# fskovbo/OptimalControlMPS

Hardware: NVIDIA B200
Metric: cost+gradient evals/s (BH N=20 chi=100) (higher is better)
Workload: dtype complex128 (f64)

## Files before the change

optimalcontrolmps_b200/csrc/decomp.cu:

```cuda
#include <cstdio>
#include <cstdlib>
#include "ocmps_internal.h"

__device__ unsigned long long g_jac_dbg[8];
__device__ double g_jac_flops[2];

namespace {

constexpr int JAC_THREADS = 512;
constexpr int JAC_EPL = 8;
constexpr int JAC_NV_SMEM = 512;
constexpr int JAC_MAX_SWEEPS = 60;
constexpr int JAC_BLOCKED_ROWS = 64;
constexpr double JAC_TOL2 = 1e-28;
constexpr double DEFLATE_REL = 1e-30;
constexpr int NV_MAX = 2048;
constexpr int BJ_C = 8;
constexpr int BJ_TPP = 4;
constexpr int BJ_MAX_ROWS = 256;
constexpr int BJ_SLOTS = BJ_MAX_ROWS / 2;
constexpr int BJ_THREADS = BJ_SLOTS * BJ_TPP;
constexpr int BJ_MAX_EPL = 8;
constexpr int BJ_MIN_CAP = 112;

// ... 1837 lines not shown
    }
#ifdef OCMPS_JAC_TRACE
    if (nv >= 24)
      printf("JTR kind %d blk %d nv %d keff %d rb %d jac %lld : rotation rounds %d, %lld clk per round; block exchanges %d, %lld clk each\n", a.kind, blk, nv,
             keff, rb, t_jac1 - t_jac0, nrounds, nrounds ? t_work / nrounds : 0ll, nxchg, nxchg ? t_xchg / nxchg : 0ll);
#endif
  }
}

__global__ void __launch_bounds__(JAC_THREADS) jacobi_rows_cluster_kernel(DecompArgs a, DecompBuffers b, int smem_elems) {
  extern __shared__ __align__(16) unsigned char smem_raw[];
  __shared__ RcShared sh;
  const int blk = (int)blockIdx.x / RC_C;
  const unsigned rank = clus::cluster_rank();
  const int keff = rot_handover_rows(b, blk, smem_elems);
  if (keff < 0) return;
  if (keff < RC_MIN_ROWS) {
    if (rank == 0) jacobi_rot_block(a, b, blk, keff, smem_raw);
    return;
  }
  cplx* Zs = reinterpret_cast<cplx*>(smem_raw);
  switch ((b.dw->blk[blk].nv + 15) >> 4) {
    case 1: rc_run<1>(a, b, blk, keff, rank, Zs, sh); break;
    case 2: rc_run<2>(a, b, blk, keff, rank, Zs, sh); break;
    case 3: rc_run<3>(a, b, blk, keff, rank, Zs, sh); break;
    case 4: rc_run<4>(a, b, blk, keff, rank, Zs, sh); break;
    case 5: rc_run<5>(a, b, blk, keff, rank, Zs, sh); break;
    case 6: rc_run<6>(a, b, blk, keff, rank, Zs, sh); break;
    case 7: rc_run<7>(a, b, blk, keff, rank, Zs, sh); break;
    default: rc_run<8>(a, b, blk, keff, rank, Zs, sh); break;
  }
}

__global__ void __launch_bounds__(1024) truncate_kernel(DecompArgs a, DecompBuffers b, TruncParams tp) {
  __shared__ double cP[NV_MAX];
  __shared__ double sSorted[NV_MAX];
  __shared__ short cQ[NV_MAX], cI[NV_MAX], cI2[NV_MAX];
  __shared__ unsigned char sKeep[NV_MAX];
  __shared__ int sBlkOff[OCMPS_MAX_BLK + 1];
  __shared__ double sWarp[32];
  __shared__ int sWarpCnt[33];
  __shared__ double s_docut, s_kept;
  __shared__ int s_nfinal;
  DecompWork* w = b.dw;
  const int nv = w->nvtot;
  const int nblocks = w->nblocks;
  const int tid = threadIdx.x, lane = tid & 31, warp = tid >> 5;
  for (int i = tid; i < nblocks; i += blockDim.x) sBlkOff[i] = w->blk[i].p_off;
  if (tid == 0) { s_nfinal = 0; s_docut = 0.0; }
  const int i0 = 2 * tid, i1 = i0 + 1;
  const double p0 = i0 < nv ? b.P[i0] : 0.0, p1 = i1 < nv ? b.P[i1] : 0.0;
  const int f0 = p0 > 0.0, f1 = p1 > 0.0;
  int incl = f0 + f1;
#pragma unroll
  for (int o = 1; o < 32; o <<= 1) { const int up = __shfl_up_sync(0xffffffffu, incl, o); if (lane >= o) incl += up; }
  if (lane == 31) sWarpCnt[warp + 1] = incl;
  if (tid == 0) sWarpCnt[0] = 0;
  __syncthreads();
  if (warp == 0) {
    int v = sWarpCnt[lane + 1];
#pragma unroll
    for (int o = 1; o < 32; o <<= 1) { const int up = __shfl_up_sync(0xffffffffu, v, o); if (lane >= o) v += up; }
    sWarpCnt[lane + 1] = v;
  }
  __syncthreads();
  const int nnz = sWarpCnt[32];
  {
    int k = sWarpCnt[warp] + incl - f0 - f1;
    if (f0) { cP[k] = p0; cQ[k] = (short)b.vecq[i0]; cI[k] = (short)i0; ++k; }
    if (f1) { cP[k] = p1; cQ[k] = (short)b.vecq[i1]; cI[k] = (short)i1; }
  }
  __syncthreads();
  {
    int tpe = 1;
    while (tpe < 8 && nnz * tpe * 2 <= (int)blockDim.x) tpe *= 2;
    const int sub = tid & (tpe - 1);
    for (int k0 = 0; k0 < nnz; k0 += (int)blockDim.x / tpe) {
      const int k = k0 + tid / tpe;
      const bool in = k < nnz;
      const double pk = in ? cP[k] : 0.0;
      int rank = 0;
      if (in)
        for (int j = sub; j < nnz; j += tpe) {
          const double pj = cP[j];
          rank += (pj > pk) || (pj == pk && j < k);
        }
      for (int o = 1; o < tpe; o <<= 1) rank += __shfl_xor_sync(0xffffffffu, rank, o);
      if (in && sub == 0) sSorted[rank] = pk;
    }
  }
  __syncthreads();
  const int origm = nv;
  const int e0 = nnz - 1 - 2 * tid, e1 = e0 - 1;
  const double v0 = e0 >= 0 ? sSorted[e0] : 0.0, v1 = e1 >= 0 ? sSorted[e1] : 0.0;
  {
    double run = v0 + v1;
#pragma unroll
    for (int o = 1; o < 32; o <<= 1) { const double up = __shfl_up_sync(0xffffffffu, run, o); if (lane >= o) run += up; }
    if (lane == 31) sWarp[warp] = run;
    __syncthreads();
    if (warp == 0) {
      double ws = sWarp[lane];
#pragma unroll
// ... 17 lines not shown
      best = nmax > 0 ? nmax : 0;
    } else {
      const int lim = nmax < nnz - 1 ? nmax : nnz - 1;
      for (int n = tid; n <= lim; n += blockDim.x)
        if (n < tp.minm || sSorted[n] >= cut) best = n > best ? n : best;
      if (tp.minm - 1 > best && tp.minm - 1 <= nmax) best = tp.minm - 1;
    }
    if (best > 0) atomicMax(&s_nfinal, best);
  }
  __syncthreads();
  {
    const int m = s_nfinal + 1;
    if (tid == 0) { sWarp[0] = 0.0; sWarp[1] = 0.0; }
    __syncthreads();
    if (e0 == m) sWarp[0] = v0;
    if (e1 == m) sWarp[0] = v1;
    if (e0 == m - 1) sWarp[1] = v0;
    if (e1 == m - 1) sWarp[1] = v1;
    __syncthreads();
    if (tid == 0) {
      double docut = 0.0;
      if (origm == 1) {
        docut = sWarp[1] / 2.0;
      } else if (origm > 1 && m < origm) {
        const double pm = sWarp[0], pm1 = sWarp[1];
        docut = (pm + pm1) / 2.0;
        if (fabs(pm - pm1) < 1e-3 * pm1) docut += 1e-3 * pm1;
      }
      s_docut = docut;
    }
    __syncthreads();
  }
  const double docut = s_docut;
  {
    const int ka = 2 * tid, kb = ka + 1;
    const int fa = ka < nnz && cP[ka] > docut, fb = kb < nnz && cP[kb] > docut;
    if (ka < nnz) sKeep[ka] = (unsigned char)fa;
    if (kb < nnz) sKeep[kb] = (unsigned char)fb;
    int inc = fa + fb;
#pragma unroll
    for (int o = 1; o < 32; o <<= 1) { const int up = __shfl_up_sync(0xffffffffu, inc, o); if (lane >= o) inc += up; }
    __syncthreads();
    if (lane == 31) sWarpCnt[warp + 1] = inc;
    if (tid == 0) sWarpCnt[0] = 0;
    __syncthreads();
    if (warp == 0) {
      int v = sWarpCnt[lane + 1];
#pragma unroll
      for (int o = 1; o < 32; o <<= 1) { const int up = __shfl_up_sync(0xffffffffu, v, o); if (lane >= o) v += up; }
      sWarpCnt[lane + 1] = v;
    }
    __syncthreads();
    const int base = sWarpCnt[warp] + inc - fa - fb;
    if (ka < nnz) cI2[ka] = (short)base;
    if (kb < nnz) cI2[kb] = (short)(base + fa);
  }
  __syncthreads();
  const int total = sWarpCnt[32];
  int* inv_blk = b.pos + NV_MAX;
  int* inv_v = b.pos + 2 * NV_MAX;
  double part = 0.0;
  for (int k = tid; k < nnz; k += blockDim.x) {
    if (!sKeep[k]) continue;
    const int qk = cQ[k];
    const double pk = cP[k];
    int rank = 0, j = k - 1;
    for (; j >= 0 && cQ[j] == qk; --j) rank += sKeep[j] && cP[j] >= pk;
    const int pos0 = cI2[j + 1];
    for (j = k + 1; j < nnz && cQ[j] == qk; ++j) rank += sKeep[j] && cP[j] > pk;
    const int pos = pos0 + rank;
    if (pos < tp.cap) {
      const int i = cI[k];
      a.qNew[pos] = qk;
      int bi = 0;
      while (bi + 1 < nblocks && sBlkOff[bi + 1] <= i) ++bi;
      inv_blk[pos] = bi;
      inv_v[pos] = i - sBlkOff[bi];
      part += pk;
    }
  }
  {
#pragma unroll
    for (int o = 16; o > 0; o >>= 1) part += __shfl_xor_sync(0xffffffffu, part, o);
    __syncthreads();
    if (lane == 0) sWarp[warp] = part;
    __syncthreads();
    if (tid == 0) {
      double t = 0.0;
      for (int i = 0; i < 32; ++i) t += sWarp[i];
      s_kept = t;
    }
    __syncthreads();
  }
  if (tid == 0) {
    int k = total;
    if (k == 0 && nv > 0) {
      k = 1;
      a.qNew[0] = b.vecq[0];
      inv_blk[0] = 0;
      inv_v[0] = 0;
    }
    if (k > tp.cap) { atomicOr(b.status, OCMPS_ST_CAPACITY); k = tp.cap; }
    w->newdim = k;
    *a.dimNew = k;
    const double kept = s_kept;
    double scale = 1.0;
    if (tp.normalize) {
      const double nrm = sqrt(kept);
      if (nrm > 1e-16) scale = 1.0 / nrm;
    }
    w->scale = scale;
    const int n = w->n, m = w->m;
    GemmDesc g1;
    g1.pad = 0;
    g1.A = g1.B = nullptr; g1.C = nullptr; g1.M = g1.N = g1.K = 0; g1.lda = g1.ldb = g1.ldc = 1; g1.opA = g1.opB = 0;
    if (a.kind == DK_ORTH_LEFT) {
      const int far = a.D * (*a.dimNb);
      g1.A = a.partner; g1.opA = 0; g1.lda = m;
      g1.B = a.nb_in; g1.opB = 0; g1.ldb = far;
      g1.C = a.nb_out; g1.ldc = far; g1.M = k; g1.N = far; g1.K = m;
    } else if (a.kind == DK_ORTH_RIGHT) {
      const int far = a.D * (*a.dimNb);
      g1.A = a.nb_in; g1.opA = 0; g1.lda = n;
      g1.B = a.partner; g1.opB = 0; g1.ldb = k;
      g1.C = a.nb_out; g1.ldc = k; g1.M = far; g1.N = k; g1.K = n;
    }
    b.descs[1] = g1;
  }
}

constexpr int BUILD_THREADS = 512;
__global__ void __launch_bounds__(BUILD_THREADS) build_factors_kernel(DecompArgs a, DecompBuffers b) {
  extern __shared__ __align__(16) unsigned char bsm[];
  __shared__ double red[BUILD_THREADS / 32];
  __shared__ double s_inv;
  const DecompWork* w = b.dw;
  const int k = w->newdim;
  const int kk = blockIdx.x;
  if (kk >= k) return;
  const int n = w->n, m = w->m, ld = w->ld, mode = w->mode;
  const int* comp_blk = b.comp_idx + NV_MAX;
  const int* comp_rank = b.comp_idx + 2 * NV_MAX;
  const int* vec_blk = b.vec_idx + NV_MAX;
  const int* vec_rank = b.vec_idx + 2 * NV_MAX;
  const int bi = b.pos[NV_MAX + kk], j = b.pos[2 * NV_MAX + kk];
  const DecompBlock B = w->blk[bi];
  const int nv = B.nv, len = B.len;
  const cplx* Zj = b.ywork + B.ws_off + (size_t)j * nv;
  const double sigma = sqrt(b.P[B.p_off + j]) * w->scale;
  cplx* zs = reinterpret_cast<cplx*>(bsm);
  cplx* out = zs + nv;
  int* vidx = reinterpret_cast<int*>(out + len);
  int* cidx = vidx + nv;
  const int tid = threadIdx.x, lane = tid & 31, wp = tid >> 5;
  constexpr int NW = BUILD_THREADS / 32;
  for (int v = tid; v < nv; v += BUILD_THREADS) { zs[v] = Zj[v]; vidx[v] = b.vec_idx[B.vec_off + v]; }
  for (int c = tid; c < len; c += BUILD_THREADS) cidx[c] = b.comp_idx[B.comp_off + c];
  __syncthreads();
  double part = 0.0;
  if (mode == 0) {
    for (int c = wp; c < len; c += NW) {
      const cplx* row = a.X + (size_t)cidx[c] * ld;
      double sr = 0.0, si = 0.0;
      for (int v0 = 0; v0 < nv; v0 += 128) {
        cplx x[4];
#pragma unroll
        for (int u = 0; u < 4; ++u) {
          const int v = v0 + lane + 32 * u;
          x[u] = make_double2(0.0, 0.0);
          if (v < nv) x[u] = row[vidx[v]];
        }
#pragma unroll
        for (int u = 0; u < 4; ++u) {
          const int v = v0 + lane + 32 * u;
          if (v < nv) {
            const cplx z = zs[v];
            sr += x[u].x * z.x + x[u].y * z.y;
            si += x[u].y * z.x - x[u].x * z.y;
          }
        }
      }
      sr = warp_sum(sr); si = warp_sum(si);
      if (lane == 0) { out[c] = make_double2(sr, si); part += sr * sr + si * si; }
    }
  } else {
    const int cl = lane & 7, g = lane >> 3;
    for (int c0 = 8 * wp; c0 < len; c0 += 8 * NW) {
      const int c = c0 + cl;
      const bool in = c < len;
      const cplx* colp = a.X + (in ? cidx[c] : 0);
      double sr = 0.0, si = 0.0;
      if (in) {
#pragma unroll 4
        for (int v = g; v < nv; v += 4) {
          const cplx x = colp[(size_t)vidx[v] * ld], z = zs[v];
          sr += x.x * z.x + x.y * z.y;
          si += x.y * z.x - x.x * z.y;
        }
      }
      sr += __shfl_xor_sync(0xffffffffu, sr, 8);  si += __shfl_xor_sync(0xffffffffu, si, 8);
      sr += __shfl_xor_sync(0xffffffffu, sr, 16); si += __shfl_xor_sync(0xffffffffu, si, 16);
      if (in && g == 0) { out[c] = make_double2(sr, si); part += sr * sr + si * si; }
    }
  }
  part = warp_sum(part);
  if ((tid & 31) == 0) red[tid >> 5] = part;
  __syncthreads();
  if (tid == 0) {
    double t = 0.0;
    for (int i = 0; i < BUILD_THREADS / 32; ++i) t += red[i];
    s_inv = t > 0.0 ? rsqrt(t) : 0.0;
  }
  __syncthreads();
  const double inv = s_inv;
  const int ncomp = mode == 0 ? n : m, nvec = mode == 0 ? m : n;
  for (int c = tid; c < ncomp; c += BUILD_THREADS) {
    cplx v = make_double2(0.0, 0.0);
    if (comp_blk[c] == bi) { const cplx o = out[comp_rank[c]]; v = make_double2(o.x * inv, o.y * inv); }
    if (mode == 0) a.iso[(size_t)c * k + kk] = v; else a.iso[(size_t)kk * m + c] = v;
  }
  if (a.qNb != nullptr && (a.kind == DK_ORTH_LEFT || a.kind == DK_ORTH_RIGHT)) {
    const int D = a.D, chiFar = *a.dimNb, qj = B.q;
    if (a.kind == DK_ORTH_LEFT) {
      const long long far = (long long)D * chiFar;
      for (int r = tid; r < chiFar; r += BUILD_THREADS) {
        const int sx = a.qNb[r] - qj;
        double ar = 0.0, ai = 0.0;
        if (sx >= 0 && sx < D) {
          const cplx* col = a.nb_in + (long long)sx * chiFar + r;
#pragma unroll 4
          for (int t = 0; t < nv; ++t) {
            const cplx z = zs[t], x = col[(long long)vidx[t] * far];
            ar += z.x * x.x - z.y * x.y;
            ai += z.x * x.y + z.y * x.x;
          }
        }
        for (int sp = 0; sp < D; ++sp)
          a.nb_out[(long long)kk * far + (long long)sp * chiFar + r] = sp == sx ? make_double2(ar * sigma, ai * sigma) : make_double2(0.0, 0.0);
      }
    } else {
      for (int l = tid; l < chiFar; l += BUILD_THREADS) {
        const int sx = qj - a.qNb[l];
        double ar = 0.0, ai = 0.0;
        if (sx >= 0 && sx < D) {
          const cplx* row = a.nb_in + ((long long)l * D + sx) * n;
#pragma unroll 4
          for (int t = 0; t < nv; ++t) {
            const cplx z = zs[t], x = row[vidx[t]];
            ar += z.x * x.x - z.y * x.y;
            ai += z.x * x.y + z.y * x.x;
          }
        }
        for (int sp = 0; sp < D; ++sp)
          a.nb_out[((long long)l * D + sp) * k + kk] = sp == sx ? make_double2(ar * sigma, ai * sigma) : make_double2(0.0, 0.0);
      }
    }
    return;
  }
  for (int v = tid; v < nvec; v += BUILD_THREADS) {
    cplx o = make_double2(0.0, 0.0);
    if (vec_blk[v] == bi) { const cplx z = zs[vec_rank[v]]; o = make_double2(z.x * sigma, z.y * sigma); }
    if (mode == 0) a.partner[(size_t)kk * m + v] = o; else a.partner[(size_t)v * k + kk] = o;
  }
}

constexpr int NORM_CTAS = 32;
constexpr int NORM_THREADS = 256;

__device__ __forceinline__ void norm_partial_body(const cplx* x, long long count, double* partial) {
  __shared__ double red[NORM_THREADS];
  double s = 0.0;
  for (long long e = blockIdx.x * (long long)NORM_THREADS + threadIdx.x; e < count; e += (long long)NORM_CTAS * NORM_THREADS) {
    cplx u = x[e];
    s += u.x * u.x + u.y * u.y;
  }
  red[threadIdx.x] = s;
  __syncthreads();
  for (int o = NORM_THREADS / 2; o > 0; o >>= 1) {
    if ((int)threadIdx.x < o) red[threadIdx.x] += red[threadIdx.x + o];
    __syncthreads();
  }
  if (threadIdx.x == 0) partial[blockIdx.x] = red[0];
}
__device__ __forceinline__ double norm_total(const double* partial) {
  double s = 0.0;
  for (int i = 0; i < NORM_CTAS; ++i) s += partial[i];
  return s;
// ... 198 lines not shown
```

optimalcontrolmps_b200/csrc/engine.cu:

```cuda
#include <cmath>
#include <complex>
#include <cstdio>
#include <cstring>
#include <cstdlib>
#include <algorithm>
#include <string>
#include <atomic>
#include <chrono>
#include <map>
#include <mutex>
#include <tuple>
#include <thread>
#include <vector>

#include "ocmps_internal.h"
#include "../../include/ocmps.h"

std::atomic<long long> g_ocmps_launches{0};

namespace {

thread_local std::string g_err;

int fail(int code, const std::string& msg) {
// ... 169 lines not shown
  for (int j = 0; j < L; ++j) m->cur[j] = 0;
  { static std::atomic<long long> next_serial{1}; m->serial = next_serial++; }
  CK(cudaStreamSynchronize(cudaStreamLegacy));
  *out = m;
  return OCMPS_OK;
}

void free_mps(ocmps_mps* m) {
  if (!m) return;
  if (m->ctx) {
    std::lock_guard<std::mutex> lock(m->ctx->mu);
    m->ctx->dead_mps.push_back(m->serial);
  }
  cudaFree(m->arena[0]); cudaFree(m->arena[1]); cudaFree(m->d_dims); cudaFree(m->d_q);
  delete m;
}

int alloc_ws(ocmps_ctx* ctx, int L, int D, int cap, bool with_work, Workspace** out, bool high_priority = false) {
  Workspace* w = new Workspace();
  w->ctx = ctx; w->L = L; w->D = D; w->cap = cap;
  CK(cudaSetDevice(ctx->dev));
  int prio_lo = 0, prio_hi = 0;
  cudaDeviceGetStreamPriorityRange(&prio_lo, &prio_hi);
  const int prio = high_priority ? prio_hi : prio_lo;
  CK(cudaStreamCreateWithPriority(&w->stream, cudaStreamNonBlocking, prio));
  const size_t nD = (size_t)cap * D;
  CK(cudaMalloc(&w->theta, sizeof(cplx) * nD * nD));
  CK(cudaMalloc(&w->cbuf, sizeof(cplx) * (size_t)cap * cap));
  CK(cudaMalloc(&w->db.dw, sizeof(DecompWork)));
  CK(cudaMalloc(&w->db.vec_idx, sizeof(int) * 3 * NV_MAX));
  CK(cudaMalloc(&w->db.comp_idx, sizeof(int) * 3 * NV_MAX));
  CK(cudaMalloc(&w->db.vecq, sizeof(int) * NV_MAX));
  CK(cudaMalloc(&w->db.P, sizeof(double) * NV_MAX));
  CK(cudaMalloc(&w->db.pos, sizeof(int) * 3 * NV_MAX));
  const size_t ywhalf = nD * cap + (size_t)cap * 16 * OCMPS_MAX_BLK;
  CK(cudaMalloc(&w->db.ywork, sizeof(cplx) * 2 * ywhalf));
  w->db.ywork_half = (long long)ywhalf;
  CK(cudaMalloc(&w->db.scratch_d, sizeof(double) * 8 * NV_MAX));
  CK(cudaMalloc(&w->db.descs, sizeof(GemmDesc) * 4));
  CK(cudaMalloc(&w->db.partial, sizeof(double) * 64));
  CK(cudaMalloc(&w->d_norm, sizeof(double) * 4));
  CK(cudaMalloc(&w->d_params, sizeof(StepParams)));
  CK(cudaMalloc(&w->d_status, sizeof(int)));
  CK(cudaMemset(w->d_status, 0, sizeof(int)));
  w->db.status = w->d_status;
  w->db2 = w->db;
  CK(cudaMalloc(&w->db2.dw, sizeof(DecompWork)));
  CK(cudaMalloc(&w->db2.vec_idx, sizeof(int) * 3 * NV_MAX));
  CK(cudaMalloc(&w->db2.comp_idx, sizeof(int) * 3 * NV_MAX));
  CK(cudaMalloc(&w->db2.vecq, sizeof(int) * NV_MAX));
  CK(cudaMalloc(&w->db2.P, sizeof(double) * NV_MAX));
  CK(cudaMalloc(&w->db2.pos, sizeof(int) * 3 * NV_MAX));
  CK(cudaMalloc(&w->db2.ywork, sizeof(cplx) * 2 * ywhalf));
  CK(cudaMalloc(&w->db2.scratch_d, sizeof(double) * 8 * NV_MAX));
  CK(cudaMalloc(&w->db2.descs, sizeof(GemmDesc) * 4));
  CK(cudaStreamCreateWithPriority(&w->side, cudaStreamNonBlocking, prio));
  CK(cudaEventCreateWithFlags(&w->ev_trunc, cudaEventDisableTiming));
  CK(cudaEventCreateWithFlags(&w->ev_setup, cudaEventDisableTiming));
  CK(cudaStreamCreateWithPriority(&w->fork.stream, cudaStreamNonBlocking, prio));
  CK(cudaEventCreateWithFlags(&w->fork.ev_fork, cudaEventDisableTiming));
  CK(cudaEventCreateWithFlags(&w->fork.ev_first, cudaEventDisableTiming));
  CK(cudaEventCreateWithFlags(&w->fork.ev_join, cudaEventDisableTiming));
  if (with_work) {
    int rc = alloc_mps(ctx, L, D, cap, &w->work);
    if (rc) return rc;
  }
  *out = w;
  return OCMPS_OK;
}

int ensure_overlap_bufs(Workspace* w, int batch, int capA, int capB) {
  const long long es = 2LL * capA * capB, ts = 2LL * capA * w->D * capB;
  if (w->obatch >= batch && w->e_stride >= es && w->t_stride >= ts) return OCMPS_OK;
  cudaFree(w->E[0]); cudaFree(w->E[1]); cudaFree(w->T); cudaFree(w->odescs); cudaFree(w->d_out);
  w->obatch = std::max(batch, w->obatch);
  w->e_stride = std::max(es, w->e_stride); w->t_stride = std::max(ts, w->t_stride);
  CK(cudaMalloc(&w->E[0], sizeof(cplx) * w->e_stride * w->obatch));
  CK(cudaMalloc(&w->E[1], sizeof(cplx) * w->e_stride * w->obatch));
  CK(cudaMalloc(&w->T, sizeof(cplx) * w->t_stride * w->obatch));
  CK(cudaMalloc(&w->odescs, sizeof(GemmDesc) * 3 * w->obatch));
  CK(cudaMalloc(&w->d_out, sizeof(cplx) * w->obatch));
  return OCMPS_OK;
}

int ensure_energy_bufs(Workspace* w, int batch, int nch, int cap) {
  auto& b = w->en;
  const long long es = (long long)nch * cap * cap, ts = (long long)nch * cap * w->D * cap;
  b.e_stride = es; b.t_stride = ts;
  if (b.e_elems >= es * batch && b.t_elems >= ts * batch && b.ndescs >= (1LL + nch) * batch && b.batch >= batch) return OCMPS_OK;
  cudaFree(b.E[0]); cudaFree(b.E[1]); cudaFree(b.T); cudaFree(b.Tm); cudaFree(b.descs); cudaFree(b.uc); cudaFree(b.out);
  b.E[0] = b.E[1] = b.T = b.Tm = nullptr; b.descs = nullptr; b.uc = b.out = nullptr;
  b.e_elems = std::max(b.e_elems, es * batch); b.t_elems = std::max(b.t_elems, ts * batch);
  b.ndescs = std::max(b.ndescs, (1LL + nch) * batch); b.batch = std::max(b.batch, batch);
  CK(cudaMalloc(&b.E[0], sizeof(cplx) * b.e_elems));
  CK(cudaMalloc(&b.E[1], sizeof(cplx) * b.e_elems));
  CK(cudaMalloc(&b.T, sizeof(cplx) * b.t_elems));
  CK(cudaMalloc(&b.Tm, sizeof(cplx) * b.t_elems));
  CK(cudaMalloc(&b.descs, sizeof(GemmDesc) * b.ndescs));
  CK(cudaMalloc(&b.uc, sizeof(double) * 2 * b.batch));
  CK(cudaMalloc(&b.out, sizeof(double) * 3 * b.batch));
  return OCMPS_OK;
}

void free_ws(Workspace* w) {
  if (!w) return;
  cudaFree(w->theta); cudaFree(w->cbuf); cudaFree(w->db.dw); cudaFree(w->db.vec_idx); cudaFree(w->db.comp_idx);
  cudaFree(w->db.vecq); cudaFree(w->db.P); cudaFree(w->db.pos); cudaFree(w->db.ywork); cudaFree(w->db.descs);
  cudaFree(w->db.partial); cudaFree(w->d_norm); cudaFree(w->db.scratch_d); cudaFree(w->d_params);
  cudaFree(w->db2.dw); cudaFree(w->db2.vec_idx); cudaFree(w->db2.comp_idx); cudaFree(w->db2.vecq); cudaFree(w->db2.P);
  cudaFree(w->db2.pos); cudaFree(w->db2.ywork); cudaFree(w->db2.scratch_d); cudaFree(w->db2.descs);
  if (w->side) cudaStreamDestroy(w->side);
  if (w->fork.stream) cudaStreamDestroy(w->fork.stream);
  if (w->fork.ev_fork) cudaEventDestroy(w->fork.ev_fork);
  if (w->fork.ev_first) cudaEventDestroy(w->fork.ev_first);
  if (w->fork.ev_join) cudaEventDestroy(w->fork.ev_join);
  if (w->ev_trunc) cudaEventDestroy(w->ev_trunc);
  if (w->ev_setup) cudaEventDestroy(w->ev_setup);
  for (auto& kv : w->graphs) if (kv.second.exec) cudaGraphExecDestroy(kv.second.exec);
  if (w->psiH) w->psiH->ctx = nullptr;
  free_mps(w->psiH);
  if (w->tmpK) w->tmpK->ctx = nullptr;
  free_mps(w->tmpK);
  if (w->rowstore) { cudaFree(w->rowstore->data); cudaFree(w->rowstore->dims); cudaFree(w->rowstore->q); delete w->rowstore; }
  cudaFree(w->E[0]); cudaFree(w->E[1]); cudaFree(w->T); cudaFree(w->odescs); cudaFree(w->d_out);
  cudaFree(w->en.E[0]); cudaFree(w->en.E[1]); cudaFree(w->en.T); cudaFree(w->en.Tm); cudaFree(w->en.descs); cudaFree(w->en.uc);
  cudaFree(w->en.out);
  cudaFree(w->d_status); cudaFree(w->d_div);
  if (w->work) w->work->ctx = nullptr;
  if (w->big) w->big->ctx = nullptr;
  free_mps(w->work); free_mps(w->big);
  if (w->bigws) free_ws(w->bigws);
  if (w->stream) cudaStreamDestroy(w->stream);
  if (w->ovl) cudaStreamDestroy(w->ovl);
  delete w;
}

struct WsLease {
  ocmps_ctx* ctx = nullptr;
  std::vector<Workspace*> ws;
  WsLease() = default;
  WsLease(const WsLease&) = delete;
  WsLease& operator=(const WsLease&) = delete;
  ~WsLease() { release(); }
// ... 142 lines not shown
        emit_position(ops, lim, ni2, L);
      }
      if (i2 == ni1 || i1 == ni2) from_left = false;
    } else {
      ops.push_back({1, i1, gk, 1});
      lim.l = i1 - 1;
      lim.r = i1 + 1;
      lim.touch(i1);
      emit_position(ops, lim, 1, L);
    }
  }
  lim.touch(1);
  ops.push_back({0, 1, 1, 0});
  ops.push_back({3, 1, 0, 0});
  return ops;
}

struct StepTrace {
  bool on = false;
  std::vector<std::pair<int, cudaEvent_t>> marks;
  void mark(int phase, cudaStream_t s) {
    if (!on) return;
    cudaEvent_t e = nullptr;
    cudaEventCreate(&e);
    cudaEventRecord(e, s);
    marks.push_back({phase, e});
  }
};
static StepTrace g_trace;
static bool step_trace_enabled() {
  static const bool v = [] { const char* e = getenv("OCMPS_STEP_TRACE"); return e && e[0] == '1'; }();
  return v;
}
enum { TR_START = 0, TR_MERGE, TR_SETUP, TR_SVD_GATE, TR_SVD_ORTH, TR_TRUNC, TR_BUILD, TR_OTHER, TR_NPHASE };

void run_decomp(Workspace* ws, const DecompArgs& a, const TruncParams& tp, int capV, int capC, int capK, cudaStream_t s,
                DecompBuffers* dbp = nullptr, bool setup_done = false, const DecompArgs* next = nullptr, DecompBuffers* db_next = nullptr) {
  DecompBuffers& db = dbp ? *dbp : ws->db;
  if (!setup_done) { launch_decomp_setup(a, db, s); g_trace.mark(TR_SETUP, s); }
  size_t need = (size_t)capV * capC * sizeof(cplx);
  need = std::max(need, (size_t)std::min(capV, capC) * (size_t)(((capV + 15) / 16) * 16) * sizeof(cplx));
  size_t smem = std::min(need, JAC_SMEM_LIMIT);
  if (smem < 1024) smem = 1024;
  int nblk = std::min(std::min(OCMPS_MAX_BLK, std::max(capV, capC) + a.D), ws->ctx->qmax.load() + a.D + 1);
  const bool need_global = need > JAC_SMEM_LIMIT;
  static const double rank_scale = [] { const char* e = getenv("OCMPS_RANK_TOL_SCALE"); return e ? atof(e) : 1e-6; }();
  double rank_tol = rank_scale * tp.cutoff;
  rank_tol = std::min(rank_scale * 1e-8, std::max(1e-30, rank_tol));
  const bool long_rows = capV > 128;
  const int max_rows = std::min(capV, capC);
  launch_jacobi_blocks(a, db, nblk, smem, need_global, long_rows, rank_tol, max_rows, capV, capC, ws->spread_jacobi, s, &ws->fork);
  g_trace.mark((a.kind == DK_GATE_LEFT || a.kind == DK_GATE_RIGHT) ? TR_SVD_GATE : TR_SVD_ORTH, s);
  launch_truncate(a, db, tp, s);
  g_trace.mark(TR_TRUNC, s);
  if (next) {
    cudaEventRecord(ws->ev_trunc, s);
    cudaStreamWaitEvent(ws->side, ws->ev_trunc, 0);
    launch_decomp_setup(*next, *db_next, ws->side);
    cudaEventRecord(ws->ev_setup, ws->side);
  }
  launch_build_factors(a, db, capK, capV, capC, s);
  g_trace.mark(TR_BUILD, s);
  g_ocmps_launches += 5 + (need_global ? 1 : 0) + (long_rows ? 1 : 0);
}

void phases_of(int D, double U, double tstep, double* re, double* im, bool imag = false) {
  for (int n = 0; n < D; ++n) {
    if (imag) {
      re[n] = std::exp(-0.25 * U * tstep * (double)n * (double)(n - 1));
      im[n] = 0.0;
      continue;
    }
    const double ang = -0.25 * U * tstep * (double)n * (double)(n - 1);
    re[n] = std::cos(ang);
    im[n] = std::sin(ang);
  }
}

static bool fused_push_enabled() {
  static const bool v = [] { const char* e = getenv("OCMPS_FUSED_PUSH"); return !(e && e[0] == '0'); }();
  return v;
}

void run_step_body(ocmps_stepper* st, ocmps_mps* m, Workspace* ws, cudaStream_t s, int op_begin = 0, int op_end = 1 << 30) {
  const int D = st->D;
  const Layout& lay = m->lay;
  const StepParams* sp = ws->d_params;
  TruncParams tpg{st->cutoff, st->maxm, 1, st->rel_cutoff, 0, 1};
  TruncParams tpo{MIN_CUT, MAX_M, 1, 0, 0, 0};

  auto setup_args = [&](const Op& op) {
    DecompArgs a;
    a.D = D;
    if (op.kind == 1) {
      const int bl = op.a - 1, br = op.a + 1;
      a.kind = op.c == 0 ? DK_GATE_LEFT : DK_GATE_RIGHT;
      a.dimL = m->dim(bl); a.dimR = m->dim(br); a.qL = m->q(bl); a.qR = m->q(br);
    } else {
      const int b = op.a;
      a.kind = op.b == 0 ? DK_ORTH_LEFT : DK_ORTH_RIGHT;
      const int lo = op.b == 0 ? b - 1 : b;
      a.dimL = m->dim(lo); a.dimR = m->dim(lo + 1); a.qL = m->q(lo); a.qR = m->q(lo + 1);
    }
    a.dimNew = nullptr; a.qNew = nullptr; a.X = nullptr; a.iso = nullptr; a.partner = nullptr;
    a.nb_in = nullptr; a.nb_out = nullptr; a.dimNb = nullptr; a.qNb = nullptr;
    return a;
  };
  const bool fused_push = fused_push_enabled();
  const int op_last = std::min((int)st->ops.size(), op_end);
  int ndec = 0;
  bool pre_setup = false;
  auto pipelined_decomp = [&](int oi, const DecompArgs& a, const TruncParams& tp, int capV, int capC, int capK) {
    DecompBuffers* dbc = (ndec & 1) ? &ws->db2 : &ws->db;
    DecompBuffers* dbn = (ndec & 1) ? &ws->db : &ws->db2;
    if (pre_setup) cudaStreamWaitEvent(s, ws->ev_setup, 0);
    int on = oi + 1;
    while (on < op_last && st->ops[on].kind != 1 && st->ops[on].kind != 2) ++on;
    DecompArgs an;
    const bool has_next = on < op_last;
    if (has_next) an = setup_args(st->ops[on]);
    run_decomp(ws, a, tp, capV, capC, capK, s, dbc, pre_setup, has_next ? &an : nullptr, dbn);
    pre_setup = has_next;
    ++ndec;
    return dbc;
  };

  for (int oi = op_begin; oi < (int)st->ops.size() && oi < op_end; ++oi) {
    const Op& op = st->ops[oi];
    if (op.kind == 0) {
      const int j = op.a - 1;
      launch_site_phase(m->site(j), m->dim(j), m->dim(j + 1), D, sp, op.b, lay.capb[j] * D * lay.capb[j + 1], s);
      g_ocmps_launches += 1;
    } else if (op.kind == 1) {
      const int j1 = op.a - 1, j2 = op.a;
      const int bl = j1, bm = j1 + 1, br = j2 + 1;
      static const bool fused_merge = [] { const char* e = getenv("OCMPS_FUSED_MERGE"); return !(e && e[0] == '0'); }();
      if (fused_merge && D >= 2 && D <= 8) {
        launch_merge_gate(m->site(j1), m->site(j2), ws->theta, m->dim(bl), m->dim(bm), m->dim(br), m->q(bl), m->q(bm), m->q(br), D, sp,
                          op.b, lay.capb[bl], lay.capb[br], s);
        g_trace.mark(TR_MERGE, s);
        g_ocmps_launches -= 2;
      } else {
        launch_merge_setup(ws->db.descs + 2, m->site(j1), m->site(j2), ws->theta, m->dim(bl), m->dim(bm), m->dim(br), D, s);
        launch_zgemm(ws->db.descs + 2, 1, lay.capb[bl] * D, D * lay.capb[br], s);
        launch_gate_apply(ws->theta, m->dim(bl), m->dim(br), m->q(bl), m->q(br), D, sp, op.b, lay.capb[bl], lay.capb[br], s);
      }
      DecompArgs a;
      a.kind = op.c == 0 ? DK_GATE_LEFT : DK_GATE_RIGHT;
// ... 77 lines not shown
    if (slot < 0 || slot >= store->nslots) return fail(OCMPS_ERR_INVALID, "slot out of range");
  }
  StepParams hp;
  fill_step_params(st, from, to, forward, store, slot, hp);
  launch_set_step_params(hp, ws->d_params, s);
  g_ocmps_launches += 1;
  const Layout& lay = m->lay;
  auto body = [&]() {
    run_step_body(st, m, ws, s);
    if (store) {
      launch_pack_to_slot(m->ptrs(), lay.offs, m->d_dims, m->d_q, lay.L, lay.D, lay.cap, lay.max_site_elems, ws->d_params, ws->d_status, s);
      g_ocmps_launches += 1;
    }
  };
  if (step_trace_enabled()) {
    CK(cudaStreamSynchronize(s));
    g_trace.on = true;
    g_trace.marks.clear();
    g_trace.mark(TR_START, s);
    body();
    g_trace.mark(TR_OTHER, s);
    g_trace.on = false;
    CK(cudaStreamSynchronize(s));
    double sum[TR_NPHASE] = {0};
    int cnt[TR_NPHASE] = {0};
    for (size_t i = 1; i < g_trace.marks.size(); ++i) {
      float ms = 0.f;
      cudaEventElapsedTime(&ms, g_trace.marks[i - 1].second, g_trace.marks[i].second);
      sum[g_trace.marks[i].first] += ms;
      ++cnt[g_trace.marks[i].first];
    }
    float tot = 0.f;
    cudaEventElapsedTime(&tot, g_trace.marks.front().second, g_trace.marks.back().second);
    static const char* names[TR_NPHASE] = {"", "merge_gate", "setup", "svd(gate)", "svd(gauge)", "truncate", "build", "other"};
    fprintf(stderr, "[ocmps step] %.3f ms:", tot);
    for (int p = 1; p < TR_NPHASE; ++p) fprintf(stderr, " %s %dx %.3f |", names[p], cnt[p], sum[p]);
    fprintf(stderr, "\n");
    for (auto& m2 : g_trace.marks) cudaEventDestroy(m2.second);
    g_trace.marks.clear();
    return OCMPS_OK;
  }
  if (!graphs_enabled() || profile_is_on()) { body(); return OCMPS_OK; }
  unsigned long long parity = 0;
  for (int j = 0; j < lay.L; ++j) parity |= (unsigned long long)(m->cur[j] & 1) << j;
  auto key = std::make_tuple(st->serial, m->serial, parity, store ? 1 : 0, ws->ctx->qmax.load(), ws->spread_jacobi ? 1 : 0);
  Workspace::StepGraph& g = ws->graphs[key];
  if (g.exec) {
    for (int j = 0; j < lay.L; ++j) m->cur[j] ^= (int)((g.flips >> j) & 1ull);
    m->llim = 0; m->rlim = 2;
    g_ocmps_launches += g.launches;
    CK(cudaGraphLaunch(g.exec, s));
    return OCMPS_OK;
  }
  if (g.seen == 0) {
    g.seen = 1;
    body();
    return OCMPS_OK;
  }
  if (ws->graphs.size() > 64) {
    for (auto& kv : ws->graphs) if (kv.second.exec) cudaGraphExecDestroy(kv.second.exec);
    ws->graphs.clear();
    Workspace::StepGraph& g2 = ws->graphs[key];
    g2.seen = 1;
    body();
    return OCMPS_OK;
  }
  const long long l0 = g_ocmps_launches;
// ... 1595 lines not shown
```

optimalcontrolmps_b200/csrc/ocmps_internal.h:

```cpp
#pragma once
#include <cuda_runtime.h>
#include <stdint.h>
#include <stddef.h>

typedef double2 cplx;

#define OCMPS_MAX_L 64
#define OCMPS_MAX_D 8
#define OCMPS_MAX_Q 256
#define OCMPS_MAX_BLK 128

#define OCMPS_ST_CAPACITY   1
#define OCMPS_ST_NOCONV     2
#define OCMPS_ST_CHARGE     4
#define OCMPS_ST_TOOMANYBLK 8

struct GemmDesc {
  const cplx* A; const cplx* B; cplx* C;
  int M, N, K;
  int lda, ldb, ldc;
  int opA, opB;
  int pad;
};

// ... 36 lines not shown
struct Phases { double re[4][OCMPS_MAX_D]; double im[4][OCMPS_MAX_D]; };

#include <atomic>
extern std::atomic<long long> g_ocmps_launches;

void debug_jacobi_counters(unsigned long long* out, bool reset);
void debug_row_cluster_counters(unsigned long long* out, bool reset);
void profile_enable(bool on);
bool profile_is_on();
void profile_read(double* out);

void launch_zgemm(const GemmDesc* d_descs, int batch, int maxM, int maxN, cudaStream_t s);

enum DecompKind { DK_GATE_LEFT = 0, DK_GATE_RIGHT = 1, DK_ORTH_LEFT = 2, DK_ORTH_RIGHT = 3 };

struct DecompArgs {
  int kind;
  int D;
  const int* dimL;
  const int* dimR;
  const int* qL;
  const int* qR;
  int* dimNew;
  int* qNew;
  const cplx* X;
  cplx* iso;
  cplx* partner;
  const cplx* nb_in;
  cplx* nb_out;
  const int* dimNb;
  const int* qNb;
};

struct DecompBuffers {
  DecompWork* dw;
  int* vec_idx; int* comp_idx;
  int* vecq;
  double* P;
  int* pos;
  cplx* ywork;
  long long ywork_half;
  double* scratch_d;
  GemmDesc* descs;
  double* partial;
  int* status;
};

void launch_decomp_setup(const DecompArgs& a, const DecompBuffers& b, cudaStream_t s);
struct SvdFork { cudaStream_t stream = nullptr; cudaEvent_t ev_fork = nullptr, ev_first = nullptr, ev_join = nullptr; };
void launch_jacobi_blocks(const DecompArgs& a, const DecompBuffers& b, int nblk_launch, size_t smem_limit, bool need_global,
                          bool long_rows, double rank_tol, int max_rows, int capV, int capC, bool spread_rows, cudaStream_t s,
                          const SvdFork* fork = nullptr);
void launch_spectrum_entropy(const DecompBuffers& b, double* out, cudaStream_t s);
void launch_truncate(const DecompArgs& a, const DecompBuffers& b, const TruncParams& tp, cudaStream_t s);
void launch_build_factors(const DecompArgs& a, const DecompBuffers& b, int cap_k, int cap_vec, int cap_comp, cudaStream_t s);

void launch_merge_setup(GemmDesc* d, const cplx* A1, const cplx* A2, cplx* theta, const int* dimL, const int* dimM,
                        const int* dimR, int D, cudaStream_t s);
void launch_merge_gate(const cplx* A1, const cplx* A2, cplx* theta, const int* dimL, const int* dimM, const int* dimR,
                       const int* qL, const int* qM, const int* qR, int D, const StepParams* sp, int gate_kind, int maxL, int maxR,
                       cudaStream_t s);
void launch_gate_apply(cplx* theta, const int* dimL, const int* dimR, const int* qL, const int* qR, int D, const StepParams* sp,
                       int gate_kind, int maxL, int maxR, cudaStream_t s);
void launch_site_phase(cplx* A, const int* dimL, const int* dimR, int D, const StepParams* sp, int which, int max_elems, cudaStream_t s);
void launch_set_step_params(const StepParams& hp, StepParams* dst, cudaStream_t s);
void launch_pack_to_slot(SitePtrs src, SiteOffs offs, const int* dims, const int* q, int L, int D, int cap, int max_site_elems,
                         const StepParams* sp, int* status, cudaStream_t s);
void launch_norm_only(const cplx* x, const int* dimL, const int* dimR, int D, double* partial, double* out, int max_elems,
                      cudaStream_t s);
void launch_normalize_site(cplx* x, const int* dimL, const int* dimR, int D, double* partial, int max_elems, cudaStream_t s);

void launch_pack_copy(SitePtrs src, cplx* dst_base, SiteOffs offs, const int* dims, int L, int D, int max_site_elems, int* status,
// ... 76 lines not shown
```

Before: 0.9265.

## Precompute kept-vector state in truncate and parallelize build neighbor contractions

Truncate now hoists its global loads to the top of the kernel and builds per-charge run tables and a charge-to-block map in shared memory. This replaces the per-element linear block search and run scans with direct lookups. It writes a compact KeptState record per kept vector, so build_factors no longer chases pos/blk/P indirections. Build_factors also processes two rows per warp in mode 0, and splits the neighbor contraction across thread groups or warp lanes instead of one thread per output row. The step trace gains finer phase labels. The risks are extra shared-memory aliasing, extra barriers inside the left-orth loop, and unguarded P reads at indices up to 2*tid+1.

```diff
diff --git a/optimalcontrolmps_b200/csrc/decomp.cu b/optimalcontrolmps_b200/csrc/decomp.cu
--- a/optimalcontrolmps_b200/csrc/decomp.cu
+++ b/optimalcontrolmps_b200/csrc/decomp.cu
@@ -1893,24 +1893,38 @@
   }
 }
 
+__device__ __forceinline__ void write_kept(KeptState* r, const DecompBlock& B, int bi, int v, double p) {
+  KeptState ks;
+  ks.blk = bi; ks.v = v; ks.q = B.q; ks.nv = B.nv; ks.len = B.len;
+  ks.vec_off = B.vec_off; ks.comp_off = B.comp_off; ks.ws_off = B.ws_off; ks.w = p;
+  *r = ks;
+}
+
 __global__ void __launch_bounds__(1024) truncate_kernel(DecompArgs a, DecompBuffers b, TruncParams tp) {
   __shared__ double cP[NV_MAX];
   __shared__ double sSorted[NV_MAX];
   __shared__ short cQ[NV_MAX], cI[NV_MAX], cI2[NV_MAX];
-  __shared__ unsigned char sKeep[NV_MAX];
-  __shared__ int sBlkOff[OCMPS_MAX_BLK + 1];
   __shared__ double sWarp[32];
   __shared__ int sWarpCnt[33];
   __shared__ double s_docut, s_kept;
   __shared__ int s_nfinal;
+  DecompBlock* sBlk = reinterpret_cast<DecompBlock*>(sSorted);
+  unsigned char* sBlkOfQ = reinterpret_cast<unsigned char*>(sBlk + OCMPS_MAX_BLK);
+  short* sRunLo = reinterpret_cast<short*>(sBlkOfQ + OCMPS_MAX_Q);
+  short* sRunHi = sRunLo + OCMPS_MAX_Q;
+  static_assert(OCMPS_MAX_BLK * sizeof(DecompBlock) + OCMPS_MAX_Q * (1 + 2 * sizeof(short)) <= NV_MAX * sizeof(double), "tables fit");
   DecompWork* w = b.dw;
+  const int tid = threadIdx.x, lane = tid & 31, warp = tid >> 5;
+  const int i0 = 2 * tid, i1 = i0 + 1;
+  const double g0 = b.P[i0], g1 = b.P[i1];
+  const int q0 = b.vecq[i0], q1 = b.vecq[i1];
+  DecompBlock myBlk;
+  if (tid < OCMPS_MAX_BLK) myBlk = w->blk[tid];
+  const int chiFar = (tid == 0 && (a.kind == DK_ORTH_LEFT || a.kind == DK_ORTH_RIGHT)) ? *a.dimNb : 0;
   const int nv = w->nvtot;
   const int nblocks = w->nblocks;
-  const int tid = threadIdx.x, lane = tid & 31, warp = tid >> 5;
-  for (int i = tid; i < nblocks; i += blockDim.x) sBlkOff[i] = w->blk[i].p_off;
   if (tid == 0) { s_nfinal = 0; s_docut = 0.0; }
-  const int i0 = 2 * tid, i1 = i0 + 1;
-  const double p0 = i0 < nv ? b.P[i0] : 0.0, p1 = i1 < nv ? b.P[i1] : 0.0;
+  const double p0 = i0 < nv ? g0 : 0.0, p1 = i1 < nv ? g1 : 0.0;
   const int f0 = p0 > 0.0, f1 = p1 > 0.0;
   int incl = f0 + f1;
 #pragma unroll
@@ -1928,8 +1942,8 @@
   const int nnz = sWarpCnt[32];
   {
     int k = sWarpCnt[warp] + incl - f0 - f1;
-    if (f0) { cP[k] = p0; cQ[k] = (short)b.vecq[i0]; cI[k] = (short)i0; ++k; }
-    if (f1) { cP[k] = p1; cQ[k] = (short)b.vecq[i1]; cI[k] = (short)i1; }
+    if (f0) { cP[k] = p0; cQ[k] = (short)q0; cI[k] = (short)i0; ++k; }
+    if (f1) { cP[k] = p1; cQ[k] = (short)q1; cI[k] = (short)i1; }
   }
   __syncthreads();
   {
@@ -2013,11 +2027,15 @@
     __syncthreads();
   }
   const double docut = s_docut;
+  if (tid < nblocks) { sBlk[tid] = myBlk; sBlkOfQ[myBlk.q] = (unsigned char)tid; }
+  for (int k = tid; k < nnz; k += blockDim.x) {
+    const int q = cQ[k];
+    if (k == 0 || cQ[k - 1] != q) sRunLo[q] = (short)k;
+    if (k == nnz - 1 || cQ[k + 1] != q) sRunHi[q] = (short)(k + 1);
+  }
   {
     const int ka = 2 * tid, kb = ka + 1;
     const int fa = ka < nnz && cP[ka] > docut, fb = kb < nnz && cP[kb] > docut;
-    if (ka < nnz) sKeep[ka] = (unsigned char)fa;
-    if (kb < nnz) sKeep[kb] = (unsigned char)fb;
     int inc = fa + fb;
 #pragma unroll
     for (int o = 1; o < 32; o <<= 1) { const int up = __shfl_up_sync(0xffffffffu, inc, o); if (lane >= o) inc += up; }
@@ -2038,25 +2056,21 @@
   }
   __syncthreads();
   const int total = sWarpCnt[32];
-  int* inv_blk = b.pos + NV_MAX;
-  int* inv_v = b.pos + 2 * NV_MAX;
   double part = 0.0;
   for (int k = tid; k < nnz; k += blockDim.x) {
-    if (!sKeep[k]) continue;
+    const double pk = cP[k];
+    if (!(pk > docut)) continue;
     const int qk = cQ[k];
-    const double pk = cP[k];
-    int rank = 0, j = k - 1;
-    for (; j >= 0 && cQ[j] == qk; --j) rank += sKeep[j] && cP[j] >= pk;
-    const int pos0 = cI2[j + 1];
-    for (j = k + 1; j < nnz && cQ[j] == qk; ++j) rank += sKeep[j] && cP[j] > pk;
-    const int pos = pos0 + rank;
+    const int lo = sRunLo[qk], hi = sRunHi[qk];
+    int rank = 0;
+#pragma unroll 4
+    for (int j = lo; j < hi; ++j) { const double pj = cP[j]; rank += pj > pk || (pj == pk && j < k); }
+    const int pos = cI2[lo] + rank;
     if (pos < tp.cap) {
       const int i = cI[k];
       a.qNew[pos] = qk;
-      int bi = 0;
-      while (bi + 1 < nblocks && sBlkOff[bi + 1] <= i) ++bi;
-      inv_blk[pos] = bi;
-      inv_v[pos] = i - sBlkOff[bi];
+      const int bi = sBlkOfQ[qk];
+      write_kept(b.kept + pos, sBlk[bi], bi, i - sBlk[bi].p_off, pk);
       part += pk;
     }
   }
@@ -2078,8 +2092,7 @@
     if (k == 0 && nv > 0) {
       k = 1;
       a.qNew[0] = b.vecq[0];
-      inv_blk[0] = 0;
-      inv_v[0] = 0;
+      write_kept(b.kept, sBlk[0], 0, 0, b.P[0]);
     }
     if (k > tp.cap) { atomicOr(b.status, OCMPS_ST_CAPACITY); k = tp.cap; }
     w->newdim = k;
@@ -2096,12 +2109,12 @@
     g1.pad = 0;
     g1.A = g1.B = nullptr; g1.C = nullptr; g1.M = g1.N = g1.K = 0; g1.lda = g1.ldb = g1.ldc = 1; g1.opA = g1.opB = 0;
     if (a.kind == DK_ORTH_LEFT) {
-      const int far = a.D * (*a.dimNb);
+      const int far = a.D * chiFar;
       g1.A = a.partner; g1.opA = 0; g1.lda = m;
       g1.B = a.nb_in; g1.opB = 0; g1.ldb = far;
       g1.C = a.nb_out; g1.ldc = far; g1.M = k; g1.N = far; g1.K = m;
     } else if (a.kind == DK_ORTH_RIGHT) {
-      const int far = a.D * (*a.dimNb);
+      const int far = a.D * chiFar;
       g1.A = a.nb_in; g1.opA = 0; g1.lda = n;
       g1.B = a.partner; g1.opB = 0; g1.ldb = k;
       g1.C = a.nb_out; g1.ldc = k; g1.M = far; g1.N = k; g1.K = n;
@@ -2115,7 +2128,12 @@
   extern __shared__ __align__(16) unsigned char bsm[];
   __shared__ double red[BUILD_THREADS / 32];
   __shared__ double s_inv;
+  __shared__ cplx s_push[BUILD_THREADS];
   const DecompWork* w = b.dw;
+  const KeptState* ks = b.kept + blockIdx.x;
+  const int bi = ks->blk, j = ks->v, nv = ks->nv, len = ks->len, qj = ks->q;
+  const int vec_off = ks->vec_off, comp_off = ks->comp_off, ws_off = ks->ws_off;
+  const double wj = ks->w;
   const int k = w->newdim;
   const int kk = blockIdx.x;
   if (kk >= k) return;
@@ -2124,45 +2142,50 @@
   const int* comp_rank = b.comp_idx + 2 * NV_MAX;
   const int* vec_blk = b.vec_idx + NV_MAX;
   const int* vec_rank = b.vec_idx + 2 * NV_MAX;
-  const int bi = b.pos[NV_MAX + kk], j = b.pos[2 * NV_MAX + kk];
-  const DecompBlock B = w->blk[bi];
-  const int nv = B.nv, len = B.len;
-  const cplx* Zj = b.ywork + B.ws_off + (size_t)j * nv;
-  const double sigma = sqrt(b.P[B.p_off + j]) * w->scale;
+  const cplx* Zj = b.ywork + ws_off + (size_t)j * nv;
+  const double sigma = sqrt(wj) * w->scale;
   cplx* zs = reinterpret_cast<cplx*>(bsm);
   cplx* out = zs + nv;
   int* vidx = reinterpret_cast<int*>(out + len);
   int* cidx = vidx + nv;
   const int tid = threadIdx.x, lane = tid & 31, wp = tid >> 5;
   constexpr int NW = BUILD_THREADS / 32;
-  for (int v = tid; v < nv; v += BUILD_THREADS) { zs[v] = Zj[v]; vidx[v] = b.vec_idx[B.vec_off + v]; }
-  for (int c = tid; c < len; c += BUILD_THREADS) cidx[c] = b.comp_idx[B.comp_off + c];
+  for (int v = tid; v < nv; v += BUILD_THREADS) { zs[v] = Zj[v]; vidx[v] = b.vec_idx[vec_off + v]; }
+  for (int c = tid; c < len; c += BUILD_THREADS) cidx[c] = b.comp_idx[comp_off + c];
   __syncthreads();
   double part = 0.0;
   if (mode == 0) {
-    for (int c = wp; c < len; c += NW) {
-      const cplx* row = a.X + (size_t)cidx[c] * ld;
-      double sr = 0.0, si = 0.0;
+    for (int c0 = wp; c0 < len; c0 += 2 * NW) {
+      const int c1 = c0 + NW;
+      const cplx* row0 = a.X + (size_t)cidx[c0] * ld;
+      const cplx* row1 = a.X + (size_t)cidx[c1 < len ? c1 : c0] * ld;
+      double sr0 = 0.0, si0 = 0.0, sr1 = 0.0, si1 = 0.0;
       for (int v0 = 0; v0 < nv; v0 += 128) {
-        cplx x[4];
+        cplx x0[4], x1[4];
 #pragma unroll
         for (int u = 0; u < 4; ++u) {
           const int v = v0 + lane + 32 * u;
-          x[u] = make_double2(0.0, 0.0);
-          if (v < nv) x[u] = row[vidx[v]];
+          x0[u] = make_double2(0.0, 0.0); x1[u] = make_double2(0.0, 0.0);
+          if (v < nv) { const int vi = vidx[v]; x0[u] = row0[vi]; x1[u] = row1[vi]; }
         }
 #pragma unroll
         for (int u = 0; u < 4; ++u) {
           const int v = v0 + lane + 32 * u;
           if (v < nv) {
             const cplx z = zs[v];
-            sr += x[u].x * z.x + x[u].y * z.y;
-            si += x[u].y * z.x - x[u].x * z.y;
+            sr0 += x0[u].x * z.x + x0[u].y * z.y;
+            si0 += x0[u].y * z.x - x0[u].x * z.y;
+            sr1 += x1[u].x * z.x + x1[u].y * z.y;
+            si1 += x1[u].y * z.x - x1[u].x * z.y;
           }
         }
       }
-      sr = warp_sum(sr); si = warp_sum(si);
-      if (lane == 0) { out[c] = make_double2(sr, si); part += sr * sr + si * si; }
+      sr0 = warp_sum(sr0); si0 = warp_sum(si0);
+      sr1 = warp_sum(sr1); si1 = warp_sum(si1);
+      if (lane == 0) {
+        out[c0] = make_double2(sr0, si0); part += sr0 * sr0 + si0 * si0;
+        if (c1 < len) { out[c1] = make_double2(sr1, si1); part += sr1 * sr1 + si1 * si1; }
+      }
     }
   } else {
     const int cl = lane & 7, g = lane >> 3;
@@ -2201,39 +2224,51 @@
     if (mode == 0) a.iso[(size_t)c * k + kk] = v; else a.iso[(size_t)kk * m + c] = v;
   }
   if (a.qNb != nullptr && (a.kind == DK_ORTH_LEFT || a.kind == DK_ORTH_RIGHT)) {
-    const int D = a.D, chiFar = *a.dimNb, qj = B.q;
+    const int D = a.D, chiFar = *a.dimNb;
     if (a.kind == DK_ORTH_LEFT) {
       const long long far = (long long)D * chiFar;
-      for (int r = tid; r < chiFar; r += BUILD_THREADS) {
-        const int sx = a.qNb[r] - qj;
+      int G = 1;
+      while (G < 8 && G * 2 * chiFar <= BUILD_THREADS) G *= 2;
+      const int R = BUILD_THREADS / G;
+      const int g = tid / R, rr = tid % R;
+      for (int r0 = 0; r0 < chiFar; r0 += R) {
+        const int r = r0 + rr;
+        const int sx = r < chiFar ? a.qNb[r] - qj : -1;
         double ar = 0.0, ai = 0.0;
         if (sx >= 0 && sx < D) {
           const cplx* col = a.nb_in + (long long)sx * chiFar + r;
 #pragma unroll 4
-          for (int t = 0; t < nv; ++t) {
+          for (int t = g; t < nv; t += G) {
             const cplx z = zs[t], x = col[(long long)vidx[t] * far];
             ar += z.x * x.x - z.y * x.y;
             ai += z.x * x.y + z.y * x.x;
           }
         }
-        for (int sp = 0; sp < D; ++sp)
-          a.nb_out[(long long)kk * far + (long long)sp * chiFar + r] = sp == sx ? make_double2(ar * sigma, ai * sigma) : make_double2(0.0, 0.0);
+        s_push[tid] = make_double2(ar, ai);
+        __syncthreads();
+        if (g == 0 && r < chiFar) {
+          for (int gg = 1; gg < G; ++gg) { const cplx p = s_push[gg * R + rr]; ar += p.x; ai += p.y; }
+          for (int sp = 0; sp < D; ++sp)
+            a.nb_out[(long long)kk * far + (long long)sp * chiFar + r] = sp == sx ? make_double2(ar * sigma, ai * sigma) : make_double2(0.0, 0.0);
+        }
+        __syncthreads();
       }
     } else {
-      for (int l = tid; l < chiFar; l += BUILD_THREADS) {
+      for (int l = wp; l < chiFar; l += NW) {
         const int sx = qj - a.qNb[l];
         double ar = 0.0, ai = 0.0;
         if (sx >= 0 && sx < D) {
           const cplx* row = a.nb_in + ((long long)l * D + sx) * n;
 #pragma unroll 4
-          for (int t = 0; t < nv; ++t) {
+          for (int t = lane; t < nv; t += 32) {
             const cplx z = zs[t], x = row[vidx[t]];
             ar += z.x * x.x - z.y * x.y;
             ai += z.x * x.y + z.y * x.x;
           }
         }
-        for (int sp = 0; sp < D; ++sp)
-          a.nb_out[((long long)l * D + sp) * k + kk] = sp == sx ? make_double2(ar * sigma, ai * sigma) : make_double2(0.0, 0.0);
+        ar = warp_sum(ar); ai = warp_sum(ai);
+        if (lane < D)
+          a.nb_out[((long long)l * D + lane) * k + kk] = lane == sx ? make_double2(ar * sigma, ai * sigma) : make_double2(0.0, 0.0);
       }
     }
     return;
diff --git a/optimalcontrolmps_b200/csrc/engine.cu b/optimalcontrolmps_b200/csrc/engine.cu
--- a/optimalcontrolmps_b200/csrc/engine.cu
+++ b/optimalcontrolmps_b200/csrc/engine.cu
@@ -225,7 +225,7 @@
   CK(cudaMalloc(&w->db.comp_idx, sizeof(int) * 3 * NV_MAX));
   CK(cudaMalloc(&w->db.vecq, sizeof(int) * NV_MAX));
   CK(cudaMalloc(&w->db.P, sizeof(double) * NV_MAX));
-  CK(cudaMalloc(&w->db.pos, sizeof(int) * 3 * NV_MAX));
+  CK(cudaMalloc(&w->db.kept, sizeof(KeptState) * NV_MAX));
   const size_t ywhalf = nD * cap + (size_t)cap * 16 * OCMPS_MAX_BLK;
   CK(cudaMalloc(&w->db.ywork, sizeof(cplx) * 2 * ywhalf));
   w->db.ywork_half = (long long)ywhalf;
@@ -243,7 +243,7 @@
   CK(cudaMalloc(&w->db2.comp_idx, sizeof(int) * 3 * NV_MAX));
   CK(cudaMalloc(&w->db2.vecq, sizeof(int) * NV_MAX));
   CK(cudaMalloc(&w->db2.P, sizeof(double) * NV_MAX));
-  CK(cudaMalloc(&w->db2.pos, sizeof(int) * 3 * NV_MAX));
+  CK(cudaMalloc(&w->db2.kept, sizeof(KeptState) * NV_MAX));
   CK(cudaMalloc(&w->db2.ywork, sizeof(cplx) * 2 * ywhalf));
   CK(cudaMalloc(&w->db2.scratch_d, sizeof(double) * 8 * NV_MAX));
   CK(cudaMalloc(&w->db2.descs, sizeof(GemmDesc) * 4));
@@ -298,10 +298,10 @@
 void free_ws(Workspace* w) {
   if (!w) return;
   cudaFree(w->theta); cudaFree(w->cbuf); cudaFree(w->db.dw); cudaFree(w->db.vec_idx); cudaFree(w->db.comp_idx);
-  cudaFree(w->db.vecq); cudaFree(w->db.P); cudaFree(w->db.pos); cudaFree(w->db.ywork); cudaFree(w->db.descs);
+  cudaFree(w->db.vecq); cudaFree(w->db.P); cudaFree(w->db.kept); cudaFree(w->db.ywork); cudaFree(w->db.descs);
   cudaFree(w->db.partial); cudaFree(w->d_norm); cudaFree(w->db.scratch_d); cudaFree(w->d_params);
   cudaFree(w->db2.dw); cudaFree(w->db2.vec_idx); cudaFree(w->db2.comp_idx); cudaFree(w->db2.vecq); cudaFree(w->db2.P);
-  cudaFree(w->db2.pos); cudaFree(w->db2.ywork); cudaFree(w->db2.scratch_d); cudaFree(w->db2.descs);
+  cudaFree(w->db2.kept); cudaFree(w->db2.ywork); cudaFree(w->db2.scratch_d); cudaFree(w->db2.descs);
   if (w->side) cudaStreamDestroy(w->side);
   if (w->fork.stream) cudaStreamDestroy(w->fork.stream);
   if (w->fork.ev_fork) cudaEventDestroy(w->fork.ev_fork);
@@ -510,7 +510,8 @@
   static const bool v = [] { const char* e = getenv("OCMPS_STEP_TRACE"); return e && e[0] == '1'; }();
   return v;
 }
-enum { TR_START = 0, TR_MERGE, TR_SETUP, TR_SVD_GATE, TR_SVD_ORTH, TR_TRUNC, TR_BUILD, TR_OTHER, TR_NPHASE };
+enum { TR_START = 0, TR_MERGE, TR_SETUP, TR_SETUP_WAIT, TR_SVD_GATE, TR_SVD_ORTH, TR_TRUNC_GATE, TR_TRUNC_ORTH, TR_BUILD_GATE,
+       TR_BUILD_ORTH, TR_OTHER, TR_NPHASE };
 
 void run_decomp(Workspace* ws, const DecompArgs& a, const TruncParams& tp, int capV, int capC, int capK, cudaStream_t s,
                 DecompBuffers* dbp = nullptr, bool setup_done = false, const DecompArgs* next = nullptr, DecompBuffers* db_next = nullptr) {
@@ -528,9 +529,10 @@
   const bool long_rows = capV > 128;
   const int max_rows = std::min(capV, capC);
   launch_jacobi_blocks(a, db, nblk, smem, need_global, long_rows, rank_tol, max_rows, capV, capC, ws->spread_jacobi, s, &ws->fork);
-  g_trace.mark((a.kind == DK_GATE_LEFT || a.kind == DK_GATE_RIGHT) ? TR_SVD_GATE : TR_SVD_ORTH, s);
+  const bool gate = a.kind == DK_GATE_LEFT || a.kind == DK_GATE_RIGHT;
+  g_trace.mark(gate ? TR_SVD_GATE : TR_SVD_ORTH, s);
   launch_truncate(a, db, tp, s);
-  g_trace.mark(TR_TRUNC, s);
+  g_trace.mark(gate ? TR_TRUNC_GATE : TR_TRUNC_ORTH, s);
   if (next) {
     cudaEventRecord(ws->ev_trunc, s);
     cudaStreamWaitEvent(ws->side, ws->ev_trunc, 0);
@@ -538,7 +540,7 @@
     cudaEventRecord(ws->ev_setup, ws->side);
   }
   launch_build_factors(a, db, capK, capV, capC, s);
-  g_trace.mark(TR_BUILD, s);
+  g_trace.mark(gate ? TR_BUILD_GATE : TR_BUILD_ORTH, s);
   g_ocmps_launches += 5 + (need_global ? 1 : 0) + (long_rows ? 1 : 0);
 }
 
@@ -591,7 +593,11 @@
   auto pipelined_decomp = [&](int oi, const DecompArgs& a, const TruncParams& tp, int capV, int capC, int capK) {
     DecompBuffers* dbc = (ndec & 1) ? &ws->db2 : &ws->db;
     DecompBuffers* dbn = (ndec & 1) ? &ws->db : &ws->db2;
-    if (pre_setup) cudaStreamWaitEvent(s, ws->ev_setup, 0);
+    if (pre_setup) {
+      g_trace.mark(TR_OTHER, s);
+      cudaStreamWaitEvent(s, ws->ev_setup, 0);
+      g_trace.mark(TR_SETUP_WAIT, s);
+    }
     int on = oi + 1;
     while (on < op_last && st->ops[on].kind != 1 && st->ops[on].kind != 2) ++on;
     DecompArgs an;
@@ -735,7 +741,8 @@
     }
     float tot = 0.f;
     cudaEventElapsedTime(&tot, g_trace.marks.front().second, g_trace.marks.back().second);
-    static const char* names[TR_NPHASE] = {"", "merge_gate", "setup", "svd(gate)", "svd(gauge)", "truncate", "build", "other"};
+    static const char* names[TR_NPHASE] = {"", "merge_gate", "setup", "setup_wait", "svd(gate)", "svd(gauge)", "truncate(gate)",
+                                           "truncate(gauge)", "build(gate)", "build(gauge)", "other"};
     fprintf(stderr, "[ocmps step] %.3f ms:", tot);
     for (int p = 1; p < TR_NPHASE; ++p) fprintf(stderr, " %s %dx %.3f |", names[p], cnt[p], sum[p]);
     fprintf(stderr, "\n");
diff --git a/optimalcontrolmps_b200/csrc/ocmps_internal.h b/optimalcontrolmps_b200/csrc/ocmps_internal.h
--- a/optimalcontrolmps_b200/csrc/ocmps_internal.h
+++ b/optimalcontrolmps_b200/csrc/ocmps_internal.h
@@ -92,12 +92,19 @@
   const int* qNb;
 };
 
+struct KeptState {
+  int blk, v;
+  int q, nv, len;
+  int vec_off, comp_off, ws_off;
+  double w;
+};
+
 struct DecompBuffers {
   DecompWork* dw;
   int* vec_idx; int* comp_idx;
   int* vecq;
   double* P;
-  int* pos;
+  KeptState* kept;
   cplx* ywork;
   long long ywork_half;
   double* scratch_d;
```

After: 0.9451, median of 6. 1.02x the previous value.
